# OpenMined/PIR

Measured on AMD Instinct MI355X. Metric: PIR queries/sec (ms/query in ms_per_step), N=4096 DB=2^20 x 288B d=2, higher is better.
Workload: dtype u64; 1 GPU; N=4096, 2 RNS data primes (36,36 bit | special 37 bit), t=24 bit, DB=2^20 x 288B, d=2, dims=[162, 162], num_pt=26215, 64 queries/step (whole job), 16 in flight per GPU (BASELINE.json configs[2]); workers=16, dist_mode=single, exchange=none, parallelism=single GPU, database_copies_in_hbm=operand layout only (u64 staging released)

## Files before the change

### pir_amd/csrc/ctx.hip

```cpp
#include <hip/hip_runtime.h>
#include <ctype.h>
#include <stdint.h>
#include <stdio.h>
#include <stdlib.h>
#include <string.h>

#include <algorithm>
#include <atomic>
#include <functional>
#include <map>
#include <mutex>
#include <string>
#include <vector>

#include "../../include/pirgpu.h"
#include "ctmult.h"
#include "device_params.h"
#include "host_math.h"
#include "kernels.h"
#include "options.h"
#include "wire.h"

using namespace pirgpu;

// ... 209 lines not shown
  uint32_t scan_rpt = 0, scan_block = 0;
  bool scan_limb = false;
  uint32_t mq_nq = 4, mq_rows = 1;
  bool mq_single = false;
  uint32_t mq_single_rows = 4;
  bool mq_single_limb = false;
  uint64_t scan_npt = 0;
  bool mfma_on = false;
  MfmaGeom mg{};
  uint32_t mfma_nq = 0;
  bool mfma_single = false;
  bool scan_f64_fold = false;
  bool scan_f64_fold_batch = false;
  bool split_upper = false;
  uint64_t split_upper_words = 0;
  bool loop_transforms = false;
  uint32_t loop_min_sources = 1024;
  uint32_t fuse_mac_nodes = 128;
  bool fuse_mac_combine = false;
  bool fuse_last_level = false;
  bool last_level_ntt = false;
  bool tree40 = false;
  bool c0_ntt = false;
  bool c0_ntt_split = false;
  bool want_sel_f64 = false;
  bool sel_f64 = false;
  bool pack40 = false;
  int pack_bytes = 5;
  uint8_t* d_dbp = nullptr;
  bool packed_valid = false;
  bool staging_released = false;
  bool streamed = false;
  uint64_t stream_bands = 1;
  uint64_t db_bytes = 0, dbp_alloc = 0, mem_scratch = 0, mem_peak = 0;
  std::vector<BatchLane> lanes;
  uint64_t groups_run = 0;
  hipStream_t head_stream = nullptr;
  uint32_t head_levels = 0;
  uint32_t head_mode = 0;
  hipEvent_t ev_head_tail = nullptr;
  hipStream_t copy_stream = nullptr;
  hipEvent_t ev_fetch[2] = {nullptr, nullptr};
  hipEvent_t ev_fork = nullptr;
  hipEvent_t ev_main_join = nullptr;

  bool ctm = false;
// ... 319 lines not shown
  c->upper_blocks = (uint32_t)std::max<int64_t>(1, c->options.value(OPT_UPPER_BLOCKS, 512));
  c->upper_blocks_batch = (uint32_t)std::max<int64_t>(1, c->options.value(OPT_UPPER_BLOCKS_BATCH, 64));
  c->upper_blocks_batch = std::min(c->upper_blocks_batch, c->upper_blocks);
  c->scan_limb = true;
  for (uint32_t j = 0; j < k; ++j) c->scan_limb = c->scan_limb && (c->hp.mod[j].q >> 50) == 0;
  if (!opt_u32(c, OPT_SCAN_LIMB, 1)) c->scan_limb = false;
  c->mq_nq = 4;
  c->mq_rows = 1;
  c->mq_single = opt_u32(c, OPT_SCAN_MQ_SINGLE, 1) != 0;
  c->mq_single_rows = 4;
  c->mq_single_limb = false;
  c->scan_rpt = opt_u32(c, OPT_SCAN_ROWS, 4);
  c->scan_block = opt_u32(c, OPT_SCAN_BLOCK, 256);
  const uint32_t xblocks = (k * N / 2 + c->scan_block - 1) / c->scan_block;
  const uint32_t yblocks = (c->scan_rows + c->scan_rpt - 1) / c->scan_rpt;
  uint64_t have = (uint64_t)xblocks * std::max<uint32_t>(yblocks, 1) * c->scan_block / 256;
  uint32_t want = have >= 512 ? 1 : (uint32_t)ceil_div(1024, std::max<uint64_t>(have, 1));
  want = opt_u32(c, OPT_SCAN_NSPLIT, want);
  want = std::max<uint32_t>(1, std::min<uint32_t>(want, std::max<uint32_t>(c->scan_cols, 1)));
  c->scan_cps = (uint32_t)ceil_div(std::max<uint32_t>(c->scan_cols, 1), want);
  c->scan_nsplit = (uint32_t)ceil_div(std::max<uint32_t>(c->scan_cols, 1), c->scan_cps);
  c->fuse_last_level = opt_u32(c, OPT_FUSE_LAST, 1) != 0;
  c->fuse_mac_combine = opt_u32(c, OPT_FUSE_MAC_COMBINE, 1) != 0;
  c->last_level_ntt = opt_u32(c, OPT_LAST_NTT, 1) != 0;
  {
    const uint32_t v = opt_u32(c, OPT_C0_NTT, 0);
    c->c0_ntt = v != 0;
    c->c0_ntt_split = v >= 2;
  }
  c->want_sel_f64 = opt_u32(c, OPT_SEL_F64, 1) != 0;
  c->tree40 = opt_u32(c, OPT_TREE40, 1) != 0;
  c->fuse_mac_nodes = 128;
  c->head_levels = std::min<uint32_t>(opt_u32(c, OPT_HEAD_LEVELS, 5), 8);
  c->head_mode = std::min<uint32_t>(opt_u32(c, OPT_HEAD_MODE, 1), 2);
  c->split_upper = opt_u32(c, OPT_SPLIT_UPPER, c->logN >= 14 ? 1 : 0) != 0 && c->mode != kNttInt;
  if (c->logN >= 15) c->split_upper = true;
  c->split_upper_words = (uint64_t)opt_u32(c, OPT_SPLIT_UPPER_MB, 3072) * (1ull << 20) / 8;
  c->loop_transforms = opt_u32(c, OPT_LOOP_TRANSFORMS, 1) != 0 && c->mode != kNttInt;
  c->pack40 = opt_u32(c, OPT_PACK40, 1) != 0;
  {
    uint32_t bits = 0;
    for (uint32_t j = 0; j <= k; ++j) bits = std::max<uint32_t>(bits, 64 - (uint32_t)__builtin_clzll(c->hp.mod[j].q));
    const int need = bits <= 39 ? 5 : (bits <= 47 ? 6 : (bits <= 55 ? 7 : 8));
    int want = (int)opt_u32(c, OPT_PACK_BYTES, (uint32_t)need);
    if (want < need) want = need;
    if (c->mode == kNttInt && want != 5) want = 8;
    if (c->logN >= 15) want = 8;
    if (want > 7) c->pack40 = false;
    c->pack_bytes = c->pack40 ? want : 5;
    if (c->pack40 && c->pack_bytes == 7 && c->logN >= 14 && !opt_u32(c, OPT_TREE40_WIDE, 0)) c->tree40 = false;
    const NttOps* ops = ntt_ops_for(N, c->pack_bytes);
    if (ops != c->ops) {
      c->ops = ops;
      HIP_TRY(c->ops->configure(c->mode));
    }
  }
  bool wide_given = false;
  const int64_t wide = c->options.value(OPT_SCAN_MFMA_WIDE, 0, &wide_given);
  c->mg = mfma_geometry(c->hp, c->scan_rows, c->scan_cols, wide_given ? (int)(wide != 0) : -1,
                        opt_u32(c, OPT_SCAN_MFMA_TOP4, 1) != 0);
  c->mfma_on = opt_u32(c, OPT_SCAN_MFMA, 1) != 0 && d >= 2 && c->mg.L != 0 && c->scan_rows >= 8 && c->scan_npt > 0;
  if (c->slot_sharded && (!c->mfma_on || c->mg.nchunks != 1 || c->nslots % c->mg.NW))
    throw Fail{PIRGPU_INVALID_ARGUMENT, "a slot shard needs the int8-MFMA scan in one column chunk (d = 2, >= 8 rows, "
                                        "moduli below 2^55, at most 28 column groups)"};
  c->mfma_nq = std::max<uint32_t>(1, std::min<uint32_t>(opt_u32(c, OPT_SCAN_MFMA_NQ, kMaxMfmaQueries), kMaxMfmaQueries));
  c->mfma_single = opt_u32(c, OPT_SCAN_MFMA_SINGLE, c->mg.nchunks == 1 ? 1 : 0) != 0;
  c->scan_f64_fold = opt_u32(c, OPT_SCAN_F64_FOLD, c->mg.L >= 6 ? 1 : 0) != 0;
  c->scan_f64_fold_batch = opt_u32(c, OPT_SCAN_F64_FOLD_BATCH, 1) != 0;
  for (uint32_t j = 0; j < k; ++j) {
    c->scan_f64_fold = c->scan_f64_fold && (c->hp.mod[j].q >> 50) == 0;
    c->scan_f64_fold_batch = c->scan_f64_fold_batch && (c->hp.mod[j].q >> 50) == 0;
  }
  const uint64_t rem = c->dim_sum % N;
  c->sel_f64 = c->want_sel_f64 && c->mfma_on && c->mode != kNttInt && c->fuse_last_level && c->last_level_ntt &&
               !c->split_upper && c->dim_sum >= 2 && rem != 1 && !c->ctm;
  if (c->ctm) c->ctm_scratch_words = (uint64_t)std::max<int64_t>(1, c->options.value(OPT_CT_SCRATCH_MB, 256)) * (1ull << 20) / 8;
  c->ctm_shared_sel = c->ctm && c->options.value(OPT_CT_SHARED_SEL, ctm_shared_sel_default(c)) != 0;
  if (c->streamed && c->mfma_on) {
    const uint64_t mb = (uint64_t)std::max<int64_t>(0, c->options.value(OPT_DB_STREAM_MB, 256));
// ... 226 lines not shown
      c0ntt = true;
    }
    HIP_TRY(c->ops->ks_digit(st, c->mode, c->dp, k, cur, g, nodes, dig, c->pack40, c0_in_digit ? prod : nullptr, cur40,
                             c->loop_transforms && (uint64_t)nodes * k >= c->loop_min_sources));
    if (level_fused(j)) {
      const uint32_t next_nodes = nodes * 2;
      const bool next_last = j + 2 == logm;
      const bool next_reads40 = next_last ? (fuse_last && c->last_level_ntt && (c0ntt || ks_digit_takes_c0(next_nodes)))
                                          : (next_nodes >= fuse_from);
      const bool out40 = c->tree40 && c->pack40 && j + 1 < logm && next_reads40 && (1u << j) < (N >> ntt_log_ept((int)c->logN));
      HIP_TRY(c->ops->ks_mac_intt(st, c->mode, c->dp, k, dig, key, nodes, prod, c->pack40, k, 1));
      HIP_TRY(c->ops->ks_mac_combine(st, c->mode, c->dp, k, dig, key, prod, cur, g, nodes, 1u << j, nxt, c->pack40, cur40,
                                     out40, c0ntt ? xpow_table(c, st, 1u << j) : nullptr,
                                     c0ntt ? galois_perm_table(c, st, g) : nullptr, c->c0_ntt_split));
      cur40 = out40;
      std::swap(cur, nxt);
      level_done();
      continue;
    }
    if (cur40 && !last_ntt) throw Fail{PIRGPU_INTERNAL, "5-byte tree reached an unfused level"};
    if (c0ntt && !last_ntt) throw Fail{PIRGPU_INTERNAL, "NTT-form c0 reached an unfused level"};
    if (fuse_last && j + 1 == logm && c->last_level_ntt) {
      const uint64_t* X = xpow_table(c, st, 1u << j);
      HIP_TRY(c->ops->ks_mac_intt(st, c->mode, c->dp, k, dig, key, nodes, prod, c->pack40, k, 1));
      HIP_TRY(c->ops->ks_last_ntt(st, c->mode, c->dp, k, cur, dig, key, prod, X, g, galois_inverse(g, N), 1u << j, n, B,
                                  *sel_dst, nodes, c->pack40, sel_f64, c0_in_digit, c0ntt ? (cur40 ? 2 : 1) : 0,
                                  galois_perm_table(c, st, g)));
      return nullptr;
    }
    HIP_TRY(c->ops->ks_mac_intt(st, c->mode, c->dp, k, dig, key, nodes, prod, c->pack40, 0, k + 1));
    if (fuse_last && j + 1 == logm) {
      HIP_TRY(c->ops->ks_last_level(st, c->mode, c->dp, k, cur, prod, g, 1u << j, n, B, *sel_dst, nodes, c->pack40));
      return nullptr;
    }
    const uint32_t hi_limit = j + 1 == logm ? n * B : UINT32_MAX;
    HIP_TRY(launch_ks_combine(st, c->dp, c->mode, N, k, cur, prod, galois_inverse(g, N), nodes, 1u << j, true, hi_limit,
                              c->pack40, nxt, c->pack_bytes));
    std::swap(cur, nxt);
    if (c0_path && j + 1 < logm && level_fused(j + 1)) {
      HIP_TRY(c->ops->tree_c0_fwd(st, c->mode, c->dp, k, cur, nodes * 2));
      c0ntt = true;
    }
    level_done();
  }
  if (to) {
    to->cur = cur;
    to->cur40 = cur40;
    to->c0ntt = c0ntt;
  }
  return cur;
// ... 1039 lines not shown
  pirgpu_ctx* c = const_cast<pirgpu_ctx*>(cc);
  if (!c) return 0;
  try {
    c->use_device();
    ensure_workspace(c);
  } catch (...) {
    return 0;
  }
  return c->mfma_on && c->mfma_single ? (uint64_t)dbp_bytes(c) : held_pts(c) / c->tables * c->k * c->N * 8;
}

int pirgpu_ntt_mode(const pirgpu_ctx* c) { return c ? c->mode : -1; }

int pirgpu_arith_info(pirgpu_ctx* c, uint32_t info[8]) {
  return guarded(c, [&]() -> int {
    if (!info) return fail(c, PIRGPU_INVALID_ARGUMENT, "null info");
    ensure_workspace(c);
    info[0] = (uint32_t)c->mode;
    info[1] = c->mode == kNttF64 ? c->hp.f64_lazy_inv : 0u;
    info[2] = c->pack40 ? (uint32_t)c->pack_bytes : 8u;
    info[3] = c->tree40 && c->pack40 ? 1u : 0u;
    info[4] = c->hp.lazy_limit;
    info[5] = (c->scan_f64_fold ? 1u : 0u) | (c->scan_f64_fold_batch ? 2u : 0u) | (c->scan_limb ? 4u : 0u);
    info[6] = info[7] = 0;
    return PIRGPU_OK;
  });
}

int pirgpu_scan_info(pirgpu_ctx* c, uint32_t info[8]) {
  return guarded(c, [&]() -> int {
    if (!info) return fail(c, PIRGPU_INVALID_ARGUMENT, "null info");
    ensure_workspace(c);
    info[0] = c->mfma_on ? 1 : 0;
    info[1] = c->mfma_on ? c->mg.L : 0;
    info[2] = c->mfma_on ? c->mg.nchunks : c->scan_nsplit;
    info[3] = c->mfma_on ? c->mg.KS : 0;
    info[4] = c->mfma_on ? c->mfma_nq : (mq_usable(c) ? std::min<uint32_t>(c->mq_nq, kMaxScanQueries) : 1);
    info[5] = c->scan_rows;
    info[6] = c->scan_cols;
    info[7] = (c->mfma_on && c->mfma_single ? 1u : 0u) | (c->mfma_on && c->mg.top4 ? 2u : 0u);
    return PIRGPU_OK;
  });
}

static int load_table_items(pirgpu_ctx* c, uint32_t table, const uint8_t* items, uint64_t num_items, uint32_t bytes_per_item);

int pirgpu_db_load_items(pirgpu_ctx* c, const uint8_t* items, uint64_t num_items, uint32_t bytes_per_item) {
// ... 2187 lines not shown
```

### pir_amd/csrc/kernels.h

```cpp
#pragma once
#include <hip/hip_runtime.h>
#include <stdint.h>

#include "device_params.h"

namespace pirgpu {

constexpr int kMaxScanChunks = 16;
constexpr int kMaxMfmaQueries = 8;
constexpr int kMaxScanGroups = 16;
constexpr int kMaxSlices = 16;

constexpr uint32_t kKsWideLevel = 256;
inline bool ks_digit_takes_c0(uint32_t nodes) { return nodes >= kKsWideLevel && nodes % 8 == 0; }

struct MfmaPtrs {
  const void* p[kMaxMfmaQueries];
};

struct ScanGroups {
  uint32_t n;
  const uint8_t* sel[kMaxScanGroups];
  uint64_t* out[kMaxScanGroups];
  uint8_t nq[kMaxScanGroups];
};

struct ScanGroupsDb : ScanGroups {
  const uint8_t* db[kMaxScanGroups];
};

struct SliceMap {
  uint32_t n;
  uint32_t cut[kMaxSlices + 1];
  uint64_t off[kMaxSlices];
};

struct KeyPtrs {
// ... 20 lines not shown
                            uint32_t I_count);
  hipError_t (*upper_fused)(hipStream_t st, int mode, const DevParams* P, uint32_t k, uint32_t enc_count,
                            const uint64_t* src, const MfmaPtrs& svq, uint64_t* part, uint32_t n_rows,
                            uint32_t n_dim, uint32_t n_children_total, uint32_t sv_first, uint32_t C,
                            uint32_t chunk_len, uint32_t n_chunks, uint32_t n_queries, uint64_t src_qstride,
                            uint64_t part_qstride, bool sel_f64);
  hipError_t (*ks_last_level)(hipStream_t st, int mode, const DevParams* P, uint32_t k, const uint64_t* tree,
                              const uint64_t* prod, uint32_t galois_elt, uint32_t shift_pow, uint32_t n_items,
                              uint32_t B, const MfmaPtrs& dst, uint32_t tree_cts, bool pack40);
  hipError_t (*upper_ntt)(hipStream_t st, int mode, const DevParams* P, uint32_t k, uint32_t enc_count,
                          const uint64_t* src, uint64_t* scratch, uint32_t n_rows, uint32_t n_dim,
                          uint32_t n_children_total, uint32_t C, uint32_t b0, uint32_t blk, uint32_t n_queries,
                          uint64_t src_qstride, bool loop_source);
  hipError_t (*ks_mac_combine)(hipStream_t st, int mode, const DevParams* P, uint32_t k, const uint64_t* dig,
                               const KeyPtrs& key, const uint64_t* prod, const uint64_t* tree_in, uint32_t galois_elt,
                               uint32_t nodes, uint32_t shift_pow, uint64_t* tree_out, bool pack40, bool tin40,
                               bool tout40, const uint64_t* xpow_c0ntt,
                               const uint16_t* perm,
                               bool c0_split);
  hipError_t (*ks_last_ntt)(hipStream_t st, int mode, const DevParams* P, uint32_t k, const uint64_t* tree,
                            const uint64_t* dig, const KeyPtrs& key, uint64_t* prod, const uint64_t* xpow,
                            uint32_t galois_elt, uint32_t galois_inv, uint32_t shift_pow, uint32_t n_items, uint32_t B,
                            const MfmaPtrs& dst, uint32_t nodes, bool pack40, bool out_f64, bool c0_done, int c0_tree,
                            const uint16_t* perm);
  hipError_t (*ntt_inv_gather)(hipStream_t st, int mode, const DevParams* P, uint32_t k, const uint64_t* src,
                               uint64_t* dst, const SliceMap& map, uint32_t RC, uint32_t nq, uint32_t nq_total,
                               uint32_t q0);
  hipError_t (*tree_c0_fwd)(hipStream_t st, int mode, const DevParams* P, uint32_t k, uint64_t* tree, uint32_t cts);
};

const NttOps* ntt_ops_for(uint32_t N, int pack_bytes = 5);

hipError_t launch_ntt_reorder(hipStream_t st, uint32_t N, const uint64_t* in, uint64_t* out, uint64_t n_polys,
                              bool to_device, bool as_f64);
hipError_t launch_copy_rows(hipStream_t st, const uint64_t* src, uint64_t* dst, const uint64_t* src_idx,
                            const uint64_t* dst_idx, uint64_t n, uint64_t words, uint64_t src_stride, uint64_t dst_stride);
hipError_t launch_db_splice(hipStream_t st, const DevParams* P, uint64_t* coef, uint32_t N, const uint8_t* img,
                            const uint8_t* upd, uint64_t n, uint64_t bytes_per_pt, uint32_t item_bytes, uint32_t bits,
                            uint32_t* nonzero);
hipError_t launch_pack40x4(hipStream_t st, const uint64_t* in, uint32_t* out, uint64_t words);
hipError_t launch_unpack40x4(hipStream_t st, const uint32_t* in, uint64_t* out, uint64_t words);
hipError_t launch_ks_combine(hipStream_t st, const DevParams* P, int mode, uint32_t N, uint32_t k,
                             const uint64_t* res_in, const uint64_t* prod, uint32_t galois_inv, uint32_t nodes,
                             uint32_t shift_pow, bool expand_step, uint32_t hi_limit, bool pack40, uint64_t* res_out,
                             int pack_bytes = 5);
hipError_t launch_tree_convert(hipStream_t st, const DevParams* P, int mode, const uint64_t* in, uint64_t* out,
                               uint64_t words, bool to_tree, uint64_t chunk_words = 0, uint64_t in_stride = 0);
// ... 73 lines not shown
```

### pir_amd/csrc/ntt_kernels.hip

```cpp
#include <hip/hip_runtime.h>
#include <stdint.h>
#include <stdlib.h>

#include "device_params.h"
#include "kernels.h"
#include "ntt_core.h"

#ifndef PIRGPU_LOGN
#error "compile with -DPIRGPU_LOGN=<11..14>"
#endif

#ifndef PIRGPU_PACK_BYTES
#define PIRGPU_PACK_BYTES 5
#endif
#define PIRGPU_CAT2(a, b) a##b
#define PIRGPU_CAT(a, b) PIRGPU_CAT2(a, b)
#if PIRGPU_PACK_BYTES == 5
#define PIRGPU_OPS_NAME PIRGPU_CAT(ntt_ops_, PIRGPU_LOGN)
#define PIRGPU_DEG_NS PIRGPU_CAT(deg, PIRGPU_LOGN)
#else
#define PIRGPU_OPS_NAME PIRGPU_CAT(PIRGPU_CAT(ntt_ops_, PIRGPU_LOGN), PIRGPU_CAT(_p, PIRGPU_PACK_BYTES))
#define PIRGPU_DEG_NS PIRGPU_CAT(PIRGPU_CAT(deg, PIRGPU_LOGN), PIRGPU_CAT(p, PIRGPU_PACK_BYTES))
#endif

// ... 885 lines not shown
  if (!half_id) {
#pragma unroll
    for (int e = 0; e < EPT; ++e) x[e] = f64_norm(a[e * NT + tid] + g[e], m);
  } else {
#pragma unroll
    for (int e = 0; e < EPT; ++e) {
      const uint32_t i = e * NT + tid;
      const double d = f64_norm(a[i] - g[e], m);
      const uint32_t sraw = i + (2 * N - shift_pow);
      sd[lds_idx<R_>(sraw & (N - 1))] = (sraw & N) ? -d : d;
    }
    __syncthreads();
#pragma unroll
    for (int e = 0; e < EPT; ++e) x[e] = sd[lds_lin_base<NT, R_>(tid) + lds_lin_off<NT, R_>(e)];
    __syncthreads();
  }
  ntt_forward<MODE, LOGN, kPF>(x, smem_raw, P, j, tid);
  uint64_t* out = (uint64_t*)dst.p[q] + ((size_t)out_slot * 2 * k + comp * k + j) * N;
#pragma unroll
  for (int e = 0; e < EPT; ++e) out[e * NT + tid] = A::out(x[e], m);
}


template <int MODE, bool P40, bool OUTF64 = false, int C0T = 0>
__global__ void __launch_bounds__(NT)
ks_last_ntt_kernel(const DevParams* __restrict__ P, const uint64_t* __restrict__ dig_raw,
                   KeyPtrs keys, const uint64_t* __restrict__ prod,
                   const double* __restrict__ xpow, uint32_t galois_elt, uint32_t galois_inv, uint32_t shift_pow,
                   uint32_t n_items, uint32_t B, MfmaPtrs dst, const uint64_t* __restrict__ tree_raw,
                   const uint16_t* __restrict__ perm) {
  using A = Arith<MODE>;
  static_assert(MODE != kNttInt, "fp64 flavours only");
  double* sd = reinterpret_cast<double*>(smem_raw);
  const uint32_t tid = threadIdx.x, k = P->k, km = k + 1;
  uint32_t node = blockIdx.x, j = blockIdx.y, comp = blockIdx.z;
  if (gridDim.y == 1 && gridDim.z == 1) {
    const uint32_t xcd = blockIdx.x & 7, t = blockIdx.x >> 3;
    comp = t & 1;
    const uint32_t u = t >> 1;
    j = u % k;
    node = (u / k) * 8 + xcd;
  }
  const typename A::Mod m = A::mod(P, j);
  const uint32_t slot = node / B, q = node % B;
  double x[EPT];
  {
    const double pf = P->p_f, half = P->p_half_f;
    const size_t spoly = ((size_t)node * 2 + comp) * km + k;
    [[maybe_unused]] Hi16 hs{};
    if constexpr (P40) hs = load40f_hi(reinterpret_cast<const uint8_t*>(prod) + spoly * kPoly40, tid);
#pragma unroll
    for (int e = 0; e < EPT; ++e) {
      double sp;
      if constexpr (P40)
        sp = load40f(reinterpret_cast<const uint8_t*>(prod) + spoly * kPoly40, hs, e, tid, f64_pack_magic(pf));
      else
        sp = reinterpret_cast<const double*>(prod)[spoly * N + e * NT + tid];
      sp = sp > half ? sp - pf : sp;
      sp = sp < -half ? sp + pf : sp;
      x[e] = f64_norm(sp, m);
    }
  }
  ntt_forward<MODE, LOGN, kPF, false>(x, smem_raw, P, j, tid);
  const size_t dpoly0 = ((size_t)node * km + j) * k;
  const double magic = f64_pack_magic(m.q);
  auto load_poly = [&](const uint64_t* base, size_t poly, double (&out)[EPT], uint32_t t) {
    if constexpr (P40) {
      const uint8_t* pp = reinterpret_cast<const uint8_t*>(base) + poly * kPoly40;
      const Hi16 h = load40f_hi(pp, t);
#pragma unroll
      for (int e = 0; e < EPT; ++e) out[e] = load40f(pp, h, e, t, magic);
    } else {
#pragma unroll
      for (int e = 0; e < EPT; ++e) out[e] = reinterpret_cast<const double*>(base)[poly * N + e * NT + t];
    }
  };
  {
#pragma unroll
    for (int e = 0; e < EPT; ++e) x[e] = -x[e];
    const double* key = reinterpret_cast<const double*>(keys.p[node % keys.B]);
    for (uint32_t J = 0; J < k; ++J) {
      const double* kj = key + (((size_t)J * 2 + comp) * km + j) * N;
      double d[EPT];
      load_poly(dig_raw, dpoly0 + J, d, tid);
#pragma unroll
      for (int e = 0; e < EPT; ++e) x[e] += f64_mulmod(d[e], kj[e * NT + tid], m);
    }
    const double pinv = P->p_inv_f[j];
#pragma unroll
    for (int e = 0; e < EPT; ++e) x[e] = f64_mulmod(f64_norm(x[e], m), pinv, m);
  }
  uint32_t tid_e = tid;
  asm volatile("" : "+v"(tid_e));
  double a[EPT];
  {
    double v[EPT];
    if (comp == 0) {
      if constexpr (C0T == 0) load_poly(prod, (size_t)node * 2 * km + j, v, tid_e);
      else tree_load<C0T == 2>(tree_raw, (size_t)node * 2 * k + j, tid_e, m.q, v);
    } else {
      load_poly(dig_raw, dpoly0 + j, v, tid_e);
    }
    __syncthreads();
#pragma unroll
    for (int e = 0; e < EPT; ++e) sd[lds_lin_base<NT, R_>(tid_e) + lds_lin_off<NT, R_>(e)] = v[e];
    __syncthreads();
    const uint32_t gel = comp == 0 ? galois_elt : galois_inv;
    [[maybe_unused]] PermIdx pi{};
    if constexpr (PIRGPU_PERM_TABLE != 0) pi = load_perm(perm + (comp == 0 ? 0 : N), tid_e);
#pragma unroll
    for (int e = 0; e < EPT; ++e) {
      const double w = sd[perm_at(pi, e, tid_e, gel)];
      if (comp == 0) {
        a[e] = v[e];
        x[e] += w;
      } else {
        a[e] = w;
      }
    }
  }
  const size_t opoly = (size_t)comp * k + j;
  uint64_t* lo = (uint64_t*)dst.p[q] + ((size_t)slot * 2 * k + opoly) * N;
#pragma unroll
  for (int e = 0; e < EPT; ++e) {
    const double r = f64_canon(f64_norm(a[e] + x[e], m), m);
    if constexpr (OUTF64) reinterpret_cast<double*>(lo)[e * NT + tid_e] = r;
    else lo[e * NT + tid_e] = A::out(r, m);
  }
  if (slot + shift_pow < n_items) {
    uint64_t* hi = (uint64_t*)dst.p[q] + ((size_t)(slot + shift_pow) * 2 * k + opoly) * N;
    const double* X = xpow + (size_t)j * N;
#pragma unroll
    for (int e = 0; e < EPT; ++e) {
      const double r = f64_canon(f64_mulmod(f64_norm(a[e] - x[e], m), X[e * NT + tid_e], m), m);
      if constexpr (OUTF64) reinterpret_cast<double*>(hi)[e * NT + tid_e] = r;
      else hi[e * NT + tid_e] = A::out(r, m);
    }
  }
}

template <int MODE, bool LDS_TW = false, bool SELF64 = false>
__global__ void __launch_bounds__(NT)
upper_fused_kernel(const DevParams* __restrict__ P, const uint64_t* __restrict__ src_all, MfmaPtrs svq,
                   uint64_t* __restrict__ part_all, uint32_t n_rows, uint32_t n_dim,
                   uint32_t n_children_total, uint32_t sv_first, uint32_t C, uint32_t chunk_len,
                   uint32_t n_chunks, uint64_t src_qstride, uint64_t part_qstride) {
  using A = Arith<MODE>;
  using T = typename A::T;
  const uint32_t tid = threadIdx.x, k = P->k, E = P->enc_count;
  const uint32_t per_query = n_rows * C * n_chunks;
  const uint32_t qi = blockIdx.x / per_query, bx = blockIdx.x % per_query;
  const uint64_t* src = src_all + (size_t)qi * src_qstride;
  const uint64_t* sv = reinterpret_cast<const uint64_t*>(svq.p[qi]);
  uint64_t* part = part_all + (size_t)qi * part_qstride;
  const uint32_t chunk = bx % n_chunks;
  const uint32_t cc = (bx / n_chunks) % C;
  const uint32_t r = bx / (n_chunks * C);
  const uint32_t e_idx = blockIdx.y, jt = blockIdx.z;
  const ModConst mc = P->mod[jt];
  const typename A::Mod m = A::mod(P, jt);
  const uint32_t sp = P->enc_poly[e_idx], sj = P->enc_res[e_idx], sh = P->enc_shift[e_idx];
  const uint64_t mask = (1ull << P->enc_bits) - 1;
// ... 342 lines not shown
    PIRGPU_SET((ks_c0_ntt_kernel<MODE, true, false, true>));
    PIRGPU_SET((ks_c0_ntt_kernel<MODE, true, true, false>));
    PIRGPU_SET((ks_c0_ntt_kernel<MODE, true, true, true>));
    PIRGPU_SET((ks_digit_kernel<MODE, true, true>));
    PIRGPU_SET((ks_digit_kernel<MODE, false, false, true>));
    PIRGPU_SET((ks_digit_kernel<MODE, true, false, true>));
    PIRGPU_SET((ks_digit_kernel<MODE, true, true, true>));
    PIRGPU_SET((upper_ntt_kernel<MODE, true>));
    PIRGPU_SET((ks_last_level_kernel<MODE, false>));
    PIRGPU_SET((ks_last_level_kernel<MODE, true>));
    PIRGPU_SET((tree_c0_ntt_kernel<MODE, false>));
    PIRGPU_SET((tree_c0_ntt_kernel<MODE, true>));
    PIRGPU_SET((ks_last_ntt_kernel<MODE, false>));
    PIRGPU_SET((ks_last_ntt_kernel<MODE, true>));
    PIRGPU_SET((ks_last_ntt_kernel<MODE, false, true>));
    PIRGPU_SET((ks_last_ntt_kernel<MODE, true, true>));
    PIRGPU_SET((ks_last_ntt_kernel<MODE, false, false, 1>));
    PIRGPU_SET((ks_last_ntt_kernel<MODE, false, true, 1>));
    PIRGPU_SET((ks_last_ntt_kernel<MODE, true, false, 1>));
    PIRGPU_SET((ks_last_ntt_kernel<MODE, true, true, 1>));
    PIRGPU_SET((ks_last_ntt_kernel<MODE, true, false, 2>));
    PIRGPU_SET((ks_last_ntt_kernel<MODE, true, true, 2>));
    PIRGPU_SET((upper_fused_kernel<MODE, false, true>));
  }
#undef PIRGPU_SET
  return hipSuccess;
}

static hipError_t op_configure(int mode) {
  PIRGPU_BY_MODE(mode, return configure_mode<MODE>());
  return hipSuccess;
}

static hipError_t op_ntt_batch(hipStream_t st, int mode, const DevParams* P, uint64_t* data, uint64_t n_polys,
                               uint32_t mod_period, uint32_t mod_base, bool inverse) {
  if (inverse) {
    PIRGPU_BY_MODE(mode, hipLaunchKernelGGL((ntt_batch_kernel<MODE, true>), dim3((uint32_t)n_polys), dim3(NT),
                                            kLdsBytes, st, P, data, mod_period, mod_base));
  } else {
    PIRGPU_BY_MODE(mode, hipLaunchKernelGGL((ntt_batch_kernel<MODE, false>), dim3((uint32_t)n_polys), dim3(NT),
                                            kLdsBytes, st, P, data, mod_period, mod_base));
  }
  return hipGetLastError();
}

static hipError_t op_ntt_inv_gather(hipStream_t st, int mode, const DevParams* P, uint32_t k, const uint64_t* src,
// ... 170 lines not shown
    if (pack40)
      hipLaunchKernelGGL((ks_last_level_kernel<kNttF64, true>), grid, dim3(NT), kLdsBytes, st, P, tree, prod, galois_elt,
                         shift_pow, n_items, B, dst);
    else
      hipLaunchKernelGGL((ks_last_level_kernel<kNttF64, false>), grid, dim3(NT), kLdsBytes, st, P, tree, prod, galois_elt,
                         shift_pow, n_items, B, dst);
  } else if (mode == kNttF64Wide) {
    if (pack40)
      hipLaunchKernelGGL((ks_last_level_kernel<kNttF64Wide, true>), grid, dim3(NT), kLdsBytes, st, P, tree, prod,
                         galois_elt, shift_pow, n_items, B, dst);
    else
      hipLaunchKernelGGL((ks_last_level_kernel<kNttF64Wide, false>), grid, dim3(NT), kLdsBytes, st, P, tree, prod,
                         galois_elt, shift_pow, n_items, B, dst);
  } else {
    return hipErrorInvalidValue;
  }
  return hipGetLastError();
}

static hipError_t op_ks_last_ntt(hipStream_t st, int mode, const DevParams* P, uint32_t k, const uint64_t* tree,
                                 const uint64_t* dig, const KeyPtrs& key, uint64_t* prod, const uint64_t* xpow,
                                 uint32_t galois_elt, uint32_t galois_inv, uint32_t shift_pow, uint32_t n_items,
                                 uint32_t B, const MfmaPtrs& dst, uint32_t nodes, bool pack40, bool out_f64,
                                 bool c0_done, int c0_tree, const uint16_t* perm) {
  const dim3 g0(nodes * k);
  const dim3 grid = nodes >= kWideLevel && nodes % 8 == 0 ? dim3(nodes * k * 2) : dim3(nodes, k, 2);
  const double* X = reinterpret_cast<const double*>(xpow);
  if (c0_tree == 2 && !pack40) return hipErrorInvalidValue;
  if (PIRGPU_PERM_TABLE != 0 && !perm) return hipErrorInvalidValue;
#define PIRGPU_LAST_NTT_K(M, P40, OF, CT)                                                                          \
  hipLaunchKernelGGL((ks_last_ntt_kernel<M, P40, OF, CT>), grid, dim3(NT), kLdsBytes, st, P, dig, key, prod, X,    \
                     galois_elt, galois_inv, shift_pow, n_items, B, dst, tree, perm)
#define PIRGPU_LAST_NTT(M, P40)                                                                                    \
  do {                                                                                                             \
    if (c0_tree == 0 && !c0_done)                                                                                  \
      hipLaunchKernelGGL((tree_c0_ntt_kernel<M, P40>), g0, dim3(NT), kLdsBytes, st, P, tree, prod);                \
    if (c0_tree == 2) {                                                                                            \
      if constexpr (P40) {                                                                                         \
        if (out_f64) PIRGPU_LAST_NTT_K(M, P40, true, 2);                                                           \
        else PIRGPU_LAST_NTT_K(M, P40, false, 2);                                                                  \
      }                                                                                                            \
    } else if (c0_tree == 1) {                                                                                     \
      if (out_f64) PIRGPU_LAST_NTT_K(M, P40, true, 1);                                                             \
      else PIRGPU_LAST_NTT_K(M, P40, false, 1);                                                                    \
    } else {                                                                                                       \
      if (out_f64) PIRGPU_LAST_NTT_K(M, P40, true, 0);                                                             \
      else PIRGPU_LAST_NTT_K(M, P40, false, 0);                                                                    \
    }                                                                                                              \
  } while (0)
  if (mode == kNttF64) {
    if (pack40) PIRGPU_LAST_NTT(kNttF64, true);
    else PIRGPU_LAST_NTT(kNttF64, false);
// ... 81 lines not shown
```

### pir_amd/csrc/options.h

```cpp
#pragma once
#include <stdint.h>
#include <stdlib.h>

#include "env_gate.h"

namespace pirgpu {

enum class OptKind : uint8_t { Early, Live, Counter };

#define PIRGPU_OPTIONS(X)                                                                                              \
  X(UPPER_BLOCKS, Early,                                                                                               \
    "target workgroup count of upper_fused_kernel; its chunk partial sums are sized by it (at least 1)")              \
  X(UPPER_BLOCKS_BATCH, Early,                                                                                         \
    "the same per query in batch mode, where other queries fill the chip too: fewer chunks = fewer partial sums to "  \
    "write and fold (at most UPPER_BLOCKS: the scratch is sized for that)")                                           \
  X(SCAN_LIMB, Early,                                                                                                  \
    "64-bit scan kernels: 28-bit limb accumulators when all data moduli are below 2^50; 0 forces the generic "        \
    "128-bit accumulators")                                                                                           \
  X(SCAN_MQ_SINGLE, Early,                                                                                             \
    "0 routes single queries through scan_kernel instead of the LDS-shared scan_mq_kernel")                           \
  X(SCAN_ROWS, Early, "64-bit scan kernels: rows accumulated per thread (1, 2, 3, 4, 6, 8)")                          \
  X(SCAN_BLOCK, Early, "64-bit scan kernels: workgroup size (64 .. 256)")                                             \
  X(SCAN_NSPLIT, Early,                                                                                                \
    "64-bit scan kernels: column splits (partial sums reduced by reduce_splits_kernel); by default the columns are "  \
    "split only when whole rows cannot fill the chip (d = 1 / few rows)")                                             \
  X(FUSE_LAST, Early, "last expansion level fused with the selector NTT; 0: off")                                     \
  X(FUSE_MAC_COMBINE, Early,                                                                                           \
    "levels below the last: combine step inside the data residues' MAC + inverse-NTT kernel; 0: a separate "          \
    "ks_combine pass")                                                                                                \
  X(LAST_NTT, Early, "the fused last expansion level is carried out in the NTT domain; 0: coefficient form")          \
  X(C0_NTT, Early,                                                                                                     \
    "c0 of the expansion tree in NTT form from the first fused level on (needs the fused levels and the NTT-domain "  \
    "last level; fp64 flavours).  0: off (the default: measured -4 % as two launches, -7.6 % as one kernel, "         \
    "profiles/r06_ab_c0_ntt_*.txt), 1: both components of a level in one kernel, 2: component 0 as a launch of its "  \
    "own")                                                                                                            \
  X(SEL_F64, Early,                                                                                                    \
    "batch lanes keep their selectors as exact doubles between the last expansion level and their two consumers "     \
    "(sel_pack, upper level): no u64 round trip (fp64 flavours, MFMA scan, NTT-domain last level); 0: off")           \
  X(TREE40, Early, "expansion tree between fused wide levels as packed polynomials; 0: doubles")                      \
  X(SPLIT_UPPER, Early,                                                                                                \
    "upper level as transform-to-scratch + elementwise MAC.  Default: on from N = 16384 in the fp64 flavours, "       \
    "where the fused kernel spills; never in the integer flavour below N = 32768, always at N = 32768 (that "         \
    "degree's table has no upper_fused)")                                                                             \
  X(SPLIT_UPPER_MB, Early, "megabytes of scratch of the split upper level per lane / worker")                         \
  X(PACK40, Early, "key-switch digits and products stored packed instead of as doubles / u64; 0: off")                \
  X(PACK_BYTES, Early,                                                                                                 \
    "packed storage of the key-switch intermediates: the fp64 flavours store x + q (|x| <= q) in the fewest whole "   \
    "bytes -- 5 for q < 2^39, 6 for q < 2^47 (cfg 4: 43 / 44 bits), 7 for q < 2^55 (cfg 5: 48 / 49 bits) -- "         \
    "instead of doubles; the integer flavour knows the 5-byte form only.  5 | 6 | 7 forces a (sufficient) width, "    \
    "8 = doubles; N = 32768 always keeps u64")                                                                        \
  X(TREE40_WIDE, Early,                                                                                                \
    "1 keeps the packed tree at N >= 16384 with 7-byte residues too.  Default 0: the combine kernel that also reads " \
    "and writes the TREE packed needs 68 bytes of scratch under the 128-register cap of a 1024-thread workgroup -- "  \
// ... 133 lines not shown
```

### pir_amd/server.py

```python
from __future__ import annotations

import ctypes as C
import enum
from typing import Dict, Iterable, List, Optional, Sequence, Union

import numpy as np

from . import capi
from .parameters import PIRParameters, calculate_dimensions


class StatusCode(enum.IntEnum):
    OK = 0
    INVALID_ARGUMENT = 3
    FAILED_PRECONDITION = 9
    UNIMPLEMENTED = 12
    INTERNAL = 13


class PirGpuError(Exception):
    def __init__(self, code: int, message: str):
        super().__init__("%s: %s" % (StatusCode(code).name if code in StatusCode._value2member_map_ else code,
                                     message))
        self.code = code
# ... 612 lines not shown
        self._check(self.lib.pirgpu_reply_copy_to_device(self.db.handle, C.c_void_p(device_ptr),
                                                         self.db.reply_ct_count()))

    def reduce_fixup_device(self, device_ptr: int) -> None:
        self._check(self.lib.pirgpu_reduce_fixup_device(self.db.handle, C.c_void_p(device_ptr),
                                                        self.db.reply_ct_count()))

    def batch_scan_timings(self) -> Dict[str, float]:
        mean, mn = C.c_float(0), C.c_float(0)
        n, wgs, nq = C.c_uint32(0), C.c_uint32(0), C.c_uint32(0)
        self._check(self.lib.pirgpu_batch_scan_timings(self.db.handle, C.byref(mean), C.byref(mn), C.byref(n), C.byref(wgs),
                                                       C.byref(nq)))
        return {"mean_ms": float(mean.value), "min_ms": float(mn.value), "launches": int(n.value),
                "workgroups": int(wgs.value), "queries": int(nq.value)}

    def ntt_mode(self) -> int:
        return int(self.lib.pirgpu_ntt_mode(self.db.handle))

    def arith_info(self) -> dict:
        info = (C.c_uint32 * 8)()
        self._check(self.lib.pirgpu_arith_info(self.db.handle, info))
        return {"ntt_mode": info[0], "f64_lazy_inv": bool(info[1]), "pack_bytes": info[2], "tree40": bool(info[3]),
                "lazy_limit": info[4], "scan_f64_fold": bool(info[5] & 1), "scan_f64_fold_batch": bool(info[5] & 2),
                "scan_limb": bool(info[5] & 4)}

    def scan_bytes(self) -> int:
        return int(self.lib.pirgpu_scan_bytes(self.db.handle))

    def scan_info(self) -> dict:
        info = (C.c_uint32 * 8)()
        self._check(self.lib.pirgpu_scan_info(self.db.handle, info))
        return {"mfma": bool(info[0]), "digits": info[1], "chunks": info[2], "ksteps": info[3],
                "queries_per_pass": info[4], "rows": info[5], "cols": info[6], "single_query_mfma": bool(info[7] & 1),
                "top_digit_nibble": bool(info[7] & 2)}

    def substitute_power_x_inplace(self, ct: np.ndarray, power: int) -> np.ndarray:
        if not (isinstance(ct, np.ndarray) and ct.dtype == np.uint64 and ct.flags["C_CONTIGUOUS"]
                and ct.shape == (2, self.k, self.N)):
            raise PirGpuError(3, "ciphertext must be a contiguous uint64 array of shape [2, %d, %d]" % (self.k, self.N))
        self._check(self.lib.pirgpu_substitute_power_x(self.db.handle, _ptr(ct), power))
        return ct

    def multiply_inverse_power_of_x(self, ct, k: int) -> np.ndarray:
        ct = self._cts(ct, 3, "ciphertext")
        out = np.empty_like(ct)
        self._check(self.lib.pirgpu_multiply_inverse_power_of_x(self.db.handle, _ptr(ct), k, _ptr(out)))
        return out
# ... 23 lines not shown
```

Measured before the change: 5551 queries/s.

## Fuse special-prime key-switch product into last-level NTT kernel for small N

```diff
diff --git a/pir_amd/csrc/ctx.hip b/pir_amd/csrc/ctx.hip
--- a/pir_amd/csrc/ctx.hip
+++ b/pir_amd/csrc/ctx.hip
@@ -255,6 +255,7 @@
   bool last_level_ntt = false;
   bool tree40 = false;
   bool c0_ntt = false;
+  uint32_t ks_inline_special = 0;
   bool c0_ntt_split = false;
   bool want_sel_f64 = false;
   bool sel_f64 = false;
@@ -620,7 +621,8 @@
   c->scan_nsplit = (uint32_t)ceil_div(std::max<uint32_t>(c->scan_cols, 1), c->scan_cps);
   c->fuse_last_level = opt_u32(c, OPT_FUSE_LAST, 1) != 0;
   c->fuse_mac_combine = opt_u32(c, OPT_FUSE_MAC_COMBINE, 1) != 0;
-  c->last_level_ntt = opt_u32(c, OPT_LAST_NTT, 1) != 0;
+  const uint32_t last_ntt_form = opt_u32(c, OPT_LAST_NTT, 2);
+  c->last_level_ntt = last_ntt_form != 0;
   {
     const uint32_t v = opt_u32(c, OPT_C0_NTT, 0);
     c->c0_ntt = v != 0;
@@ -653,6 +655,10 @@
       HIP_TRY(c->ops->configure(c->mode));
     }
   }
+  c->ks_inline_special = last_ntt_form >= 2 && c->mode != kNttInt && c->pack40 && c->pack_bytes == 5 && N <= 4096 &&
+                                 c->fuse_last_level && !c->slot_sharded && !c->ctm
+                             ? 1
+                             : 0;
   bool wide_given = false;
   const int64_t wide = c->options.value(OPT_SCAN_MFMA_WIDE, 0, &wide_given);
   c->mg = mfma_geometry(c->hp, c->scan_rows, c->scan_cols, wide_given ? (int)(wide != 0) : -1,
@@ -925,10 +931,11 @@
     if (c0ntt && !last_ntt) throw Fail{PIRGPU_INTERNAL, "NTT-form c0 reached an unfused level"};
     if (fuse_last && j + 1 == logm && c->last_level_ntt) {
       const uint64_t* X = xpow_table(c, st, 1u << j);
-      HIP_TRY(c->ops->ks_mac_intt(st, c->mode, c->dp, k, dig, key, nodes, prod, c->pack40, k, 1));
+      const bool inl = c->ks_inline_special >= 1 && nodes >= fuse_from && ks_inline_special_ok(N, c->pack_bytes, nodes);
+      if (!inl) HIP_TRY(c->ops->ks_mac_intt(st, c->mode, c->dp, k, dig, key, nodes, prod, c->pack40, k, 1));
       HIP_TRY(c->ops->ks_last_ntt(st, c->mode, c->dp, k, cur, dig, key, prod, X, g, galois_inverse(g, N), 1u << j, n, B,
                                   *sel_dst, nodes, c->pack40, sel_f64, c0_in_digit, c0ntt ? (cur40 ? 2 : 1) : 0,
-                                  galois_perm_table(c, st, g)));
+                                  galois_perm_table(c, st, g), inl));
       return nullptr;
     }
     HIP_TRY(c->ops->ks_mac_intt(st, c->mode, c->dp, k, dig, key, nodes, prod, c->pack40, 0, k + 1));
@@ -2014,7 +2021,8 @@
     info[3] = c->tree40 && c->pack40 ? 1u : 0u;
     info[4] = c->hp.lazy_limit;
     info[5] = (c->scan_f64_fold ? 1u : 0u) | (c->scan_f64_fold_batch ? 2u : 0u) | (c->scan_limb ? 4u : 0u);
-    info[6] = info[7] = 0;
+    info[6] = c->ks_inline_special;
+    info[7] = 0;
     return PIRGPU_OK;
   });
 }
diff --git a/pir_amd/csrc/kernels.h b/pir_amd/csrc/kernels.h
--- a/pir_amd/csrc/kernels.h
+++ b/pir_amd/csrc/kernels.h
@@ -13,6 +13,9 @@
 
 constexpr uint32_t kKsWideLevel = 256;
 inline bool ks_digit_takes_c0(uint32_t nodes) { return nodes >= kKsWideLevel && nodes % 8 == 0; }
+inline bool ks_inline_special_ok(uint32_t N, int pack_bytes, uint32_t nodes) {
+  return N <= 4096 && pack_bytes == 5 && nodes >= 64 && nodes % 8 == 0;
+}
 
 struct MfmaPtrs {
   const void* p[kMaxMfmaQueries];
@@ -79,7 +82,8 @@
                             const uint64_t* dig, const KeyPtrs& key, uint64_t* prod, const uint64_t* xpow,
                             uint32_t galois_elt, uint32_t galois_inv, uint32_t shift_pow, uint32_t n_items, uint32_t B,
                             const MfmaPtrs& dst, uint32_t nodes, bool pack40, bool out_f64, bool c0_done, int c0_tree,
-                            const uint16_t* perm);
+                            const uint16_t* perm,
+                            bool inline_special);
   hipError_t (*ntt_inv_gather)(hipStream_t st, int mode, const DevParams* P, uint32_t k, const uint64_t* src,
                                uint64_t* dst, const SliceMap& map, uint32_t RC, uint32_t nq, uint32_t nq_total,
                                uint32_t q0);
diff --git a/pir_amd/csrc/ntt_kernels.hip b/pir_amd/csrc/ntt_kernels.hip
--- a/pir_amd/csrc/ntt_kernels.hip
+++ b/pir_amd/csrc/ntt_kernels.hip
@@ -931,6 +931,117 @@
 }
 
 
+template <int MODE, bool P40, bool OUTF64, int C0T, bool A1LOOP>
+__device__ __forceinline__ void ks_last_ntt_tail(const DevParams* __restrict__ P, const uint64_t* __restrict__ dig_raw,
+                                                 const KeyPtrs& keys, const uint64_t* __restrict__ prod,
+                                                 const double* __restrict__ xpow, uint32_t galois_elt, uint32_t galois_inv,
+                                                 uint32_t shift_pow, uint32_t n_items, uint32_t B, const MfmaPtrs& dst,
+                                                 const uint64_t* __restrict__ tree_raw, const uint16_t* __restrict__ perm,
+                                                 uint32_t node, uint32_t j, uint32_t comp, uint32_t tid, double (&x)[EPT]) {
+  using A = Arith<MODE>;
+  double* sd = reinterpret_cast<double*>(smem_raw);
+  const uint32_t k = P->k, km = k + 1;
+  const typename A::Mod m = A::mod(P, j);
+  const uint32_t slot = node / B, q = node % B;
+  const size_t dpoly0 = ((size_t)node * km + j) * k;
+  const double magic = f64_pack_magic(m.q);
+  auto load_poly = [&](const uint64_t* base, size_t poly, double (&out)[EPT], uint32_t t) {
+    if constexpr (P40) {
+      const uint8_t* pp = reinterpret_cast<const uint8_t*>(base) + poly * kPoly40;
+      const Hi16 h = load40f_hi(pp, t);
+#pragma unroll
+      for (int e = 0; e < EPT; ++e) out[e] = load40f(pp, h, e, t, magic);
+    } else {
+#pragma unroll
+      for (int e = 0; e < EPT; ++e) out[e] = reinterpret_cast<const double*>(base)[poly * N + e * NT + t];
+    }
+  };
+  {
+#pragma unroll
+    for (int e = 0; e < EPT; ++e) x[e] = -x[e];
+    const double* key = reinterpret_cast<const double*>(keys.p[node % keys.B]);
+    double d[EPT];
+    for (uint32_t Jc = 0; Jc < k; ++Jc) {
+      uint32_t J = Jc;
+      if constexpr (A1LOOP) J = Jc + 1 == k ? j : Jc + (Jc >= j ? 1u : 0u);
+      const double* kj = key + (((size_t)J * 2 + comp) * km + j) * N;
+      if constexpr (A1LOOP) {
+        double kv[EPT];
+        loadf64_rsrc(kj, tid, kv);
+        load40f_rsrc(reinterpret_cast<const uint8_t*>(dig_raw) + (dpoly0 + J) * kPoly40, tid, magic, d);
+#pragma unroll
+        for (int e = 0; e < EPT; ++e) x[e] += f64_mulmod(d[e], kv[e], m);
+      } else {
+        load_poly(dig_raw, dpoly0 + J, d, tid);
+#pragma unroll
+        for (int e = 0; e < EPT; ++e) x[e] += f64_mulmod(d[e], kj[e * NT + tid], m);
+      }
+    }
+    if constexpr (A1LOOP) {
+      if (comp != 0) {
+        __syncthreads();
+#pragma unroll
+        for (int e = 0; e < EPT; ++e) sd[lds_lin_base<NT, R_>(tid) + lds_lin_off<NT, R_>(e)] = d[e];
+      }
+    }
+    const double pinv = P->p_inv_f[j];
+#pragma unroll
+    for (int e = 0; e < EPT; ++e) x[e] = f64_mulmod(f64_norm(x[e], m), pinv, m);
+  }
+  uint32_t tid_e = tid;
+  asm volatile("" : "+v"(tid_e));
+  double a[EPT];
+  {
+    double v[EPT];
+    if (A1LOOP && comp != 0) {
+#pragma unroll
+      for (int e = 0; e < EPT; ++e) v[e] = 0.0;
+    } else {
+      if (comp == 0) {
+        if constexpr (C0T == 0) load_poly(prod, (size_t)node * 2 * km + j, v, tid_e);
+        else tree_load<C0T == 2>(tree_raw, (size_t)node * 2 * k + j, tid_e, m.q, v);
+      } else {
+        load_poly(dig_raw, dpoly0 + j, v, tid_e);
+      }
+      __syncthreads();
+#pragma unroll
+      for (int e = 0; e < EPT; ++e) sd[lds_lin_base<NT, R_>(tid_e) + lds_lin_off<NT, R_>(e)] = v[e];
+    }
+    __syncthreads();
+    const uint32_t gel = comp == 0 ? galois_elt : galois_inv;
+    [[maybe_unused]] PermIdx pi{};
+    if constexpr (PIRGPU_PERM_TABLE != 0) pi = load_perm(perm + (comp == 0 ? 0 : N), tid_e);
+#pragma unroll
+    for (int e = 0; e < EPT; ++e) {
+      const double w = sd[perm_at(pi, e, tid_e, gel)];
+      if (comp == 0) {
+        a[e] = v[e];
+        x[e] += w;
+      } else {
+        a[e] = w;
+      }
+    }
+  }
+  const size_t opoly = (size_t)comp * k + j;
+  uint64_t* lo = (uint64_t*)dst.p[q] + ((size_t)slot * 2 * k + opoly) * N;
+#pragma unroll
+  for (int e = 0; e < EPT; ++e) {
+    const double r = f64_canon(f64_norm(a[e] + x[e], m), m);
+    if constexpr (OUTF64) reinterpret_cast<double*>(lo)[e * NT + tid_e] = r;
+    else lo[e * NT + tid_e] = A::out(r, m);
+  }
+  if (slot + shift_pow < n_items) {
+    uint64_t* hi = (uint64_t*)dst.p[q] + ((size_t)(slot + shift_pow) * 2 * k + opoly) * N;
+    const double* X = xpow + (size_t)j * N;
+#pragma unroll
+    for (int e = 0; e < EPT; ++e) {
+      const double r = f64_canon(f64_mulmod(f64_norm(a[e] - x[e], m), X[e * NT + tid_e], m), m);
+      if constexpr (OUTF64) reinterpret_cast<double*>(hi)[e * NT + tid_e] = r;
+      else hi[e * NT + tid_e] = A::out(r, m);
+    }
+  }
+}
+
 template <int MODE, bool P40, bool OUTF64 = false, int C0T = 0>
 __global__ void __launch_bounds__(NT)
 ks_last_ntt_kernel(const DevParams* __restrict__ P, const uint64_t* __restrict__ dig_raw,
@@ -940,7 +1051,6 @@
                    const uint16_t* __restrict__ perm) {
   using A = Arith<MODE>;
   static_assert(MODE != kNttInt, "fp64 flavours only");
-  double* sd = reinterpret_cast<double*>(smem_raw);
   const uint32_t tid = threadIdx.x, k = P->k, km = k + 1;
   uint32_t node = blockIdx.x, j = blockIdx.y, comp = blockIdx.z;
   if (gridDim.y == 1 && gridDim.z == 1) {
@@ -951,7 +1061,6 @@
     node = (u / k) * 8 + xcd;
   }
   const typename A::Mod m = A::mod(P, j);
-  const uint32_t slot = node / B, q = node % B;
   double x[EPT];
   {
     const double pf = P->p_f, half = P->p_half_f;
@@ -971,82 +1080,96 @@
     }
   }
   ntt_forward<MODE, LOGN, kPF, false>(x, smem_raw, P, j, tid);
-  const size_t dpoly0 = ((size_t)node * km + j) * k;
-  const double magic = f64_pack_magic(m.q);
-  auto load_poly = [&](const uint64_t* base, size_t poly, double (&out)[EPT], uint32_t t) {
-    if constexpr (P40) {
-      const uint8_t* pp = reinterpret_cast<const uint8_t*>(base) + poly * kPoly40;
-      const Hi16 h = load40f_hi(pp, t);
-#pragma unroll
-      for (int e = 0; e < EPT; ++e) out[e] = load40f(pp, h, e, t, magic);
-    } else {
-#pragma unroll
-      for (int e = 0; e < EPT; ++e) out[e] = reinterpret_cast<const double*>(base)[poly * N + e * NT + t];
-    }
-  };
-  {
-#pragma unroll
-    for (int e = 0; e < EPT; ++e) x[e] = -x[e];
-    const double* key = reinterpret_cast<const double*>(keys.p[node % keys.B]);
-    for (uint32_t J = 0; J < k; ++J) {
-      const double* kj = key + (((size_t)J * 2 + comp) * km + j) * N;
-      double d[EPT];
-      load_poly(dig_raw, dpoly0 + J, d, tid);
-#pragma unroll
-      for (int e = 0; e < EPT; ++e) x[e] += f64_mulmod(d[e], kj[e * NT + tid], m);
-    }
-    const double pinv = P->p_inv_f[j];
-#pragma unroll
-    for (int e = 0; e < EPT; ++e) x[e] = f64_mulmod(f64_norm(x[e], m), pinv, m);
-  }
-  uint32_t tid_e = tid;
-  asm volatile("" : "+v"(tid_e));
-  double a[EPT];
-  {
-    double v[EPT];
-    if (comp == 0) {
-      if constexpr (C0T == 0) load_poly(prod, (size_t)node * 2 * km + j, v, tid_e);
-      else tree_load<C0T == 2>(tree_raw, (size_t)node * 2 * k + j, tid_e, m.q, v);
-    } else {
-      load_poly(dig_raw, dpoly0 + j, v, tid_e);
-    }
+  ks_last_ntt_tail<MODE, P40, OUTF64, C0T, false>(P, dig_raw, keys, prod, xpow, galois_elt, galois_inv, shift_pow, n_items, B, dst,
+                                                  tree_raw, perm, node, j, comp, tid, x);
+}
+
+#if PIRGPU_LOGN <= 12 && PIRGPU_PACK_BYTES == 5
+#define PIRGPU_INLINE_SPECIAL 1
+#else
+#define PIRGPU_INLINE_SPECIAL 0
+#endif
+#if PIRGPU_INLINE_SPECIAL
+constexpr size_t kInlineLdsBytes = kLdsBytes + (size_t)N * 4;
+
+template <int MODE>
+__device__ __forceinline__ Hi16 ks_special_stash(const DevParams* __restrict__ P, const uint64_t* __restrict__ dig_raw,
+                                                 const uint64_t* __restrict__ key_raw, uint32_t node, uint32_t comp,
+                                                 uint32_t tid) {
+  using A = Arith<MODE>;
+  const uint32_t k = P->k, km = k + 1;
+  const typename A::Mod mp = A::mod(P, k);
+  const double magic = f64_pack_magic(mp.q);
+  const size_t dpoly0 = ((size_t)node * km + k) * k;
+  const double* key = reinterpret_cast<const double*>(key_raw);
+  double x[EPT];
+#pragma unroll
+  for (int e = 0; e < EPT; ++e) x[e] = 0.0;
+  for (uint32_t J = 0; J < k; ++J) {
+    double d[EPT], kv[EPT];
+    load40f_rsrc(reinterpret_cast<const uint8_t*>(dig_raw) + (dpoly0 + J) * kPoly40, tid, magic, d);
+    loadf64_rsrc(key + (((size_t)J * 2 + comp) * km + k) * N, tid, kv);
+#pragma unroll
+    for (int e = 0; e < EPT; ++e) x[e] += f64_mulmod(d[e], kv[e], mp);
+  }
+#pragma unroll
+  for (int e = 0; e < EPT; ++e) x[e] = f64_norm(x[e], mp);
+  ntt_inverse<MODE, LOGN, kPF, false>(x, smem_raw, P, k, tid);
+  const double pf = P->p_f, half = P->p_half_f;
+  uint32_t* stash = reinterpret_cast<uint32_t*>(smem_raw + kLdsBytes);
+  uint32_t hb[EPT];
+#pragma unroll
+  for (int e = 0; e < EPT; ++e) {
+    double sp = x[e];
+    sp = sp > half ? sp - pf : sp;
+    sp = sp < -half ? sp + pf : sp;
+    uint32_t lo;
+    f64_pack40(sp, magic, lo, hb[e]);
+    stash[e * NT + tid] = lo;
+  }
+  Hi16 hs;
+  pack_hi_bytes(hb, hs.w);
+  return hs;
+}
+template <int MODE>
+__device__ __forceinline__ void ks_special_unstash(const DevParams* __restrict__ P, const Hi16& hs, uint32_t tid,
+                                                   const typename Arith<MODE>::Mod& m, double (&x)[EPT]) {
+  const double magic = f64_pack_magic(Arith<MODE>::mod(P, P->k).q);
+  const uint32_t* stash = reinterpret_cast<const uint32_t*>(smem_raw + kLdsBytes);
+#pragma unroll
+  for (int e = 0; e < EPT; ++e) {
+    const uint32_t lo = stash[e * NT + tid];
+    x[e] = f64_norm(__longlong_as_double((long long)(((uint64_t)hi_word(hs, e) << 32) | lo)) - magic, m);
+  }
+}
+
+template <int MODE, bool OUTF64, int C0T>
+__global__ void __launch_bounds__(NT) __attribute__((amdgpu_waves_per_eu(3)))
+ks_last_ntt_inline_kernel(const DevParams* __restrict__ P, const uint64_t* __restrict__ dig_raw, KeyPtrs keys,
+                          const uint64_t* __restrict__ prod, const double* __restrict__ xpow, uint32_t galois_elt,
+                          uint32_t galois_inv, uint32_t shift_pow, uint32_t n_items, uint32_t B, MfmaPtrs dst,
+                          const uint64_t* __restrict__ tree_raw, const uint16_t* __restrict__ perm) {
+  using A = Arith<MODE>;
+  static_assert(MODE != kNttInt, "fp64 flavours only");
+  const uint32_t tid = threadIdx.x, k = P->k;
+  const uint32_t xcd = blockIdx.x & 7, t = blockIdx.x >> 3;
+  const uint32_t comp = t & 1, node = (t >> 1) * 8 + xcd;
+  Hi16 hs = ks_special_stash<MODE>(P, dig_raw, keys.p[node % keys.B], node, comp, tid);
+#pragma clang loop unroll(disable)
+  for (uint32_t jj = 0; jj < k; ++jj) {
+    uint32_t tl = tid, j = jj;
+    asm volatile("" : "+v"(tl), "+s"(j));
+#pragma unroll
+    for (int g = 0; g < kHW; ++g) asm volatile("" : "+v"(hs.w[g]));
+    double x[EPT];
+    ks_special_unstash<MODE>(P, hs, tl, A::mod(P, j), x);
     __syncthreads();
-#pragma unroll
-    for (int e = 0; e < EPT; ++e) sd[lds_lin_base<NT, R_>(tid_e) + lds_lin_off<NT, R_>(e)] = v[e];
-    __syncthreads();
-    const uint32_t gel = comp == 0 ? galois_elt : galois_inv;
-    [[maybe_unused]] PermIdx pi{};
-    if constexpr (PIRGPU_PERM_TABLE != 0) pi = load_perm(perm + (comp == 0 ? 0 : N), tid_e);
-#pragma unroll
-    for (int e = 0; e < EPT; ++e) {
-      const double w = sd[perm_at(pi, e, tid_e, gel)];
-      if (comp == 0) {
-        a[e] = v[e];
-        x[e] += w;
-      } else {
-        a[e] = w;
-      }
-    }
-  }
-  const size_t opoly = (size_t)comp * k + j;
-  uint64_t* lo = (uint64_t*)dst.p[q] + ((size_t)slot * 2 * k + opoly) * N;
-#pragma unroll
-  for (int e = 0; e < EPT; ++e) {
-    const double r = f64_canon(f64_norm(a[e] + x[e], m), m);
-    if constexpr (OUTF64) reinterpret_cast<double*>(lo)[e * NT + tid_e] = r;
-    else lo[e * NT + tid_e] = A::out(r, m);
-  }
-  if (slot + shift_pow < n_items) {
-    uint64_t* hi = (uint64_t*)dst.p[q] + ((size_t)(slot + shift_pow) * 2 * k + opoly) * N;
-    const double* X = xpow + (size_t)j * N;
-#pragma unroll
-    for (int e = 0; e < EPT; ++e) {
-      const double r = f64_canon(f64_mulmod(f64_norm(a[e] - x[e], m), X[e * NT + tid_e], m), m);
-      if constexpr (OUTF64) reinterpret_cast<double*>(hi)[e * NT + tid_e] = r;
-      else hi[e * NT + tid_e] = A::out(r, m);
-    }
-  }
-}
+    ntt_forward<MODE, LOGN, kPFLoop, false>(x, smem_raw, P, j, tl);
+    ks_last_ntt_tail<MODE, true, OUTF64, C0T, true>(P, dig_raw, keys, prod, xpow, galois_elt, galois_inv, shift_pow, n_items, B,
+                                                    dst, tree_raw, perm, node, j, comp, tl, x);
+  }
+}
+#endif
 
 template <int MODE, bool LDS_TW = false, bool SELF64 = false>
 __global__ void __launch_bounds__(NT)
@@ -1435,6 +1558,17 @@
     PIRGPU_SET((ks_last_ntt_kernel<MODE, true, false, 2>));
     PIRGPU_SET((ks_last_ntt_kernel<MODE, true, true, 2>));
     PIRGPU_SET((upper_fused_kernel<MODE, false, true>));
+#if PIRGPU_INLINE_SPECIAL
+#define PIRGPU_SET_INLINE(K) \
+  if ((e = hipFuncSetAttribute((const void*)K, hipFuncAttributeMaxDynamicSharedMemorySize, (int)kInlineLdsBytes))) return e
+    PIRGPU_SET_INLINE((ks_last_ntt_inline_kernel<MODE, false, 0>));
+    PIRGPU_SET_INLINE((ks_last_ntt_inline_kernel<MODE, true, 0>));
+    PIRGPU_SET_INLINE((ks_last_ntt_inline_kernel<MODE, false, 1>));
+    PIRGPU_SET_INLINE((ks_last_ntt_inline_kernel<MODE, true, 1>));
+    PIRGPU_SET_INLINE((ks_last_ntt_inline_kernel<MODE, false, 2>));
+    PIRGPU_SET_INLINE((ks_last_ntt_inline_kernel<MODE, true, 2>));
+#undef PIRGPU_SET_INLINE
+#endif
   }
 #undef PIRGPU_SET
   return hipSuccess;
@@ -1651,12 +1785,42 @@
                                  const uint64_t* dig, const KeyPtrs& key, uint64_t* prod, const uint64_t* xpow,
                                  uint32_t galois_elt, uint32_t galois_inv, uint32_t shift_pow, uint32_t n_items,
                                  uint32_t B, const MfmaPtrs& dst, uint32_t nodes, bool pack40, bool out_f64,
-                                 bool c0_done, int c0_tree, const uint16_t* perm) {
+                                 bool c0_done, int c0_tree, const uint16_t* perm, bool inline_special) {
   const dim3 g0(nodes * k);
   const dim3 grid = nodes >= kWideLevel && nodes % 8 == 0 ? dim3(nodes * k * 2) : dim3(nodes, k, 2);
   const double* X = reinterpret_cast<const double*>(xpow);
   if (c0_tree == 2 && !pack40) return hipErrorInvalidValue;
   if (PIRGPU_PERM_TABLE != 0 && !perm) return hipErrorInvalidValue;
+  if (inline_special) {
+#if PIRGPU_INLINE_SPECIAL
+    if (!ks_inline_special_ok(N, 5, nodes) || !pack40 || (mode != kNttF64 && mode != kNttF64Wide)) return hipErrorInvalidValue;
+#define PIRGPU_LAST_INL_K(M, OF, CT)                                                                                  \
+  hipLaunchKernelGGL((ks_last_ntt_inline_kernel<M, OF, CT>), dim3(nodes * 2), dim3(NT), kInlineLdsBytes, st, P, dig,  \
+                     key, prod, X, galois_elt, galois_inv, shift_pow, n_items, B, dst, tree, perm)
+#define PIRGPU_LAST_INL(M)                                                                                            \
+  do {                                                                                                                \
+    if (c0_tree == 0 && !c0_done)                                                                                     \
+      hipLaunchKernelGGL((tree_c0_ntt_kernel<M, true>), g0, dim3(NT), kLdsBytes, st, P, tree, prod);                  \
+    if (c0_tree == 2) {                                                                                               \
+      if (out_f64) PIRGPU_LAST_INL_K(M, true, 2);                                                                     \
+      else PIRGPU_LAST_INL_K(M, false, 2);                                                                            \
+    } else if (c0_tree == 1) {                                                                                        \
+      if (out_f64) PIRGPU_LAST_INL_K(M, true, 1);                                                                     \
+      else PIRGPU_LAST_INL_K(M, false, 1);                                                                            \
+    } else {                                                                                                          \
+      if (out_f64) PIRGPU_LAST_INL_K(M, true, 0);                                                                     \
+      else PIRGPU_LAST_INL_K(M, false, 0);                                                                            \
+    }                                                                                                                 \
+  } while (0)
+    if (mode == kNttF64) PIRGPU_LAST_INL(kNttF64);
+    else PIRGPU_LAST_INL(kNttF64Wide);
+#undef PIRGPU_LAST_INL
+#undef PIRGPU_LAST_INL_K
+    return hipGetLastError();
+#else
+    return hipErrorInvalidValue;
+#endif
+  }
 #define PIRGPU_LAST_NTT_K(M, P40, OF, CT)                                                                          \
   hipLaunchKernelGGL((ks_last_ntt_kernel<M, P40, OF, CT>), grid, dim3(NT), kLdsBytes, st, P, dig, key, prod, X,    \
                      galois_elt, galois_inv, shift_pow, n_items, B, dst, tree, perm)
diff --git a/pir_amd/csrc/options.h b/pir_amd/csrc/options.h
--- a/pir_amd/csrc/options.h
+++ b/pir_amd/csrc/options.h
@@ -28,7 +28,12 @@
   X(FUSE_MAC_COMBINE, Early,                                                                                           \
     "levels below the last: combine step inside the data residues' MAC + inverse-NTT kernel; 0: a separate "          \
     "ks_combine pass")                                                                                                \
-  X(LAST_NTT, Early, "the fused last expansion level is carried out in the NTT domain; 0: coefficient form")          \
+  X(LAST_NTT, Early,                                                                                                   \
+    "the fused last expansion level is carried out in the NTT domain; 0: coefficient form; 2 (the default): from 64 "  \
+    "tree ciphertexts on its workgroups form the special-prime product themselves, one per (tree ciphertext, "         \
+    "component) looping over the data moduli, instead of reading back what a ks_mac_intt launch stored (fp64 "         \
+    "flavours, 5-byte intermediates, N <= 4096, not the slot-sharded step or ciphertext-multiplication mode; "         \
+    "elsewhere 2 means 1)")                                                                                            \
   X(C0_NTT, Early,                                                                                                     \
     "c0 of the expansion tree in NTT form from the first fused level on (needs the fused levels and the NTT-domain "  \
     "last level; fp64 flavours).  0: off (the default: measured -4 % as two launches, -7.6 % as one kernel, "         \
diff --git a/pir_amd/server.py b/pir_amd/server.py
--- a/pir_amd/server.py
+++ b/pir_amd/server.py
@@ -658,7 +658,7 @@
         self._check(self.lib.pirgpu_arith_info(self.db.handle, info))
         return {"ntt_mode": info[0], "f64_lazy_inv": bool(info[1]), "pack_bytes": info[2], "tree40": bool(info[3]),
                 "lazy_limit": info[4], "scan_f64_fold": bool(info[5] & 1), "scan_f64_fold_batch": bool(info[5] & 2),
-                "scan_limb": bool(info[5] & 4)}
+                "scan_limb": bool(info[5] & 4), "ks_inline_special": info[6]}
 
     def scan_bytes(self) -> int:
         return int(self.lib.pirgpu_scan_bytes(self.db.handle))
```

Measured after the change: 5601 queries/s, median of 6. No clear change (+0.9%).
